# bzhangGo/zero

Measured on AMD Instinct MI355X. Metric: src+tgt tokens/sec training, Transformer-base d=512 L=6, higher is better.
Workload: dtype bf16; 1 GPU; Transformer-base (d=512, L=6+6, F=2048, h=8, V=32000) training step, B=64 x (src 64 + tgt 64) tokens per GPU, dropout 0.10, label_smooth 0.1, fwd+bwd+allreduce+Adam; model_name=transformer, parallelism=dp1, hip_graph=whole step

## Files before the change

### include/zero_hip.h

```cpp
#ifndef ZERO_HIP_H_
#define ZERO_HIP_H_

#include <stddef.h>
#include <stdint.h>

#ifdef __cplusplus
extern "C" {
#endif

typedef void* zk_stream_t;

int zk_version(void);
const char* zk_last_error_string(void);

size_t zk_gemm_workspace(int M, int N, int K);
size_t zk_gemm_workspace_split(int M, int N, int splits);
int zk_gemm_parts(const void* A, const void* B, float* parts, int M, int N, int K, int lda, int ldb, int ta, int tb,
                  int splits, int* nparts_out, zk_stream_t stream);
size_t zk_gemm_add_ln_workspace(int rows, int N);
int zk_ln_epoch_bump(uint32_t* epoch, zk_stream_t stream);
int zk_gemm_add_ln(const void* A, const void* B, int M, int N, int K, int lda, int ldb, const float* bias,
                   const void* residual, int ldr, float drop_p, const uint64_t* seed, uint32_t sid, const float* gamma,
                   const float* beta, float eps, void* s_out, void* y, float* mean, float* rstd, void* slots,
                   size_t slots_bytes, const uint32_t* epoch, uint32_t site, int* err, zk_stream_t stream);
// ... 97 lines not shown
int zk_ce_fused(const float* logits, const int* ids, const float* w, float* ce_out, void* dlogits, int rows,
                int V, int ld, float label_smooth, zk_stream_t stream);
int zk_target_stats(const int* ids, float* mask, float* w, int B, int L, float loss_scale, zk_stream_t stream);
int zk_loss_reduce(const float* ce, const int* ids, float* per_sample, float* loss, int B, int L,
                   zk_stream_t stream);
int zk_make_mask(const int* ids, float* mask, int n, zk_stream_t stream);
size_t zk_batch_prep_workspace(int rows);
int zk_batch_prep(const int* src_ids, const int* tgt_ids, int B, int Ls, int Lt, int* src_rows, int* src_seg,
                  int* src_uid, int* src_n, int* tgt_rows, int* tgt_seg, int* tgt_uid, int* tgt_n, float* smask,
                  float* tmask, float* tw, float loss_scale, int max_id, void* scratch, size_t scratch_bytes,
                  zk_stream_t stream);
int zk_copy_many(void* const* dsts, const void* const* srcs, const size_t* nbytes, int n, zk_stream_t stream);
int zk_all_equal(const int* ids, int n, int value, int* flag, zk_stream_t stream);

int zk_aan_fwd(const void* x, const float* mask, void* cat, int B, int L, int H, int use_mask,
               zk_stream_t stream);
int zk_add_bf16(void* out, int ldo, const void* a, int lda, const void* b, int ldb, int rows, int cols,
                zk_stream_t stream);
int zk_aan_bwd(const void* dcat, const void* dxg, const void* dyg, const void* ds, const float* mask, void* dx,
               int B, int L, int H, int use_mask, zk_stream_t stream);
int zk_aan_gate_fwd(const void* z, const void* cat, void* out, int rows, int H, zk_stream_t stream);
int zk_aan_gate_bwd(const void* dg, const void* z, const void* cat, void* dz, void* dxg, void* dyg, int rows,
                    int H, zk_stream_t stream);

size_t zk_norm_workspace(void);
int zk_l2norm(const float* x, size_t n, float scale, float* out, void* workspace, size_t ws_bytes,
              zk_stream_t stream);
int zk_adam(float* p, const float* g, float* m, float* v, void* shadow_bf16, size_t n, float* hyper,
            float* pnorm_out, void* workspace, size_t ws_bytes, zk_stream_t stream);
size_t zk_adam_step_workspace(void);
int zk_adam_step(float* p, const float* g, float* m, float* v, void* shadow_bf16, size_t n, float* hyper,
                 float* pnorm_out, uint64_t* seed, int norm_free, const int* skip_word, void* workspace, size_t ws_bytes,
                 zk_stream_t stream);
int zk_norm_flag(float* hyper, zk_stream_t stream);
int zk_cast_f32_bf16(const float* x, void* y, size_t n, zk_stream_t stream);
int zk_cast_bf16_f32(const void* x, float* y, size_t n, zk_stream_t stream);
int zk_zero(void* p, size_t bytes, zk_stream_t stream);
size_t zk_rows_payload_bytes(int R, int H, int bf16);
int zk_transpose_bf16(const void* src, int ld_src, void* dst, int ld_dst, int rows, int cols, zk_stream_t stream);
int zk_rows_pack(float* dtable, const int* uid, const int* n_uniq_dev, void* out, int R, int H, int out_bf16,
                 int clear_rows, zk_stream_t stream);
int zk_rows_scatter_add(float* dtable, const void* payload, int R, int H, int in_bf16, int vocab_rows,
                        zk_stream_t stream);
uint32_t zk_crc32c(const void* data, size_t n, uint32_t crc);
int zk_spin(uint32_t usec, zk_stream_t stream);
int zk_tune(int key, int value);
int zk_ema(float* ema, const float* p, const float* hyper, size_t n, zk_stream_t stream);
int zk_axpby_f32(float* y, const float* x, float a, float b, size_t n, zk_stream_t stream);

int zk_comm_available(void);
int zk_comm_unique_id(void* id128);
int zk_comm_init(const void* id128, int nranks, int rank, void** comm_out);
int zk_comm_destroy(void* comm);
int zk_comm_size(const void* comm);
int zk_comm_allreduce(void* comm, void* buf, size_t count, int dtype, zk_stream_t stream);
int zk_comm_allreduce_multi(void* comm, void* const* bufs, const size_t* counts, int n, int dtype,
                            zk_stream_t stream);
int zk_comm_allgather(void* comm, const void* send, void* recv, size_t count, int dtype, zk_stream_t stream);
int zk_flag_add(void* flag, zk_stream_t stream);
int zk_flag_wait(const void* flag, unsigned long long target, int* err, zk_stream_t stream);

int zk_dropout_mask(float* out, size_t n, float drop_p, const uint64_t* seed, uint32_t sid, zk_stream_t stream);
int zk_seed_advance(uint64_t* seed, uint64_t inc, zk_stream_t stream);

size_t zk_beam_topk_workspace(int B, int K, int k2);
int zk_beam_topk(const float* logits, const float* prev_log_probs, float* topk_scores, int* topk_index, int B,
// ... 152 lines not shown
```

### zero_amd/csrc/zk_elem.hip

```cpp
#include "zk_common.h"
#include "zk_ln_dev.h"
#ifdef ZK_STEP_STAMPS
__device__ unsigned long long zk_step_stamp_buf[2 * 4096];
__device__ unsigned int zk_step_stamp_n[2];
extern "C" int zk_step_stamps_read(unsigned long long* out, unsigned int* n2) {
  if (hipMemcpyFromSymbol(out, HIP_SYMBOL(zk_step_stamp_buf), sizeof(unsigned long long) * 2 * 4096) != hipSuccess) return 1;
  return (int)hipMemcpyFromSymbol(n2, HIP_SYMBOL(zk_step_stamp_n), sizeof(unsigned int) * 2);
}
extern "C" int zk_step_stamps_reset(void) {
  unsigned int z[2] = {0, 0};
  return (int)hipMemcpyToSymbol(HIP_SYMBOL(zk_step_stamp_n), z, sizeof(z));
}
#endif
#include <cstring>
#include <mutex>
#include <stdarg.h>
#include <stdio.h>
#include <unordered_map>

thread_local char zk_err_buf[512] = {0};
int zk_set_error(int code, const char* fmt, ...) {
  va_list ap;
  va_start(ap, fmt);
  vsnprintf(zk_err_buf, sizeof(zk_err_buf), fmt, ap);
// ... 1058 lines not shown
    dx[j] = g[j] * si;
    dy[j] = g[j] * sf;
  }
  *reinterpret_cast<uint4*>(dz + r * 2 * H + c) = pack8(dzi);
  *reinterpret_cast<uint4*>(dz + r * 2 * H + H + c) = pack8(dzf);
  *reinterpret_cast<uint4*>(dxg + r * H + c) = pack8(dx);
  *reinterpret_cast<uint4*>(dyg + r * H + c) = pack8(dy);
}

__global__ void __launch_bounds__(256) k_sumsq_partial(const float* __restrict__ x, size_t n,
                                                       float* __restrict__ partials) {
  __shared__ float sm[8];
  float acc = 0.f;
  const size_t n4 = n / 4;
  const float4* x4 = reinterpret_cast<const float4*>(x);
  for (size_t i = (size_t)blockIdx.x * 256 + threadIdx.x; i < n4; i += (size_t)gridDim.x * 256) {
    const float4 v = x4[i];
    acc += v.x * v.x + v.y * v.y + v.z * v.z + v.w * v.w;
  }
  for (size_t i = n4 * 4 + (size_t)blockIdx.x * 256 + threadIdx.x; i < n; i += (size_t)gridDim.x * 256)
    acc += x[i] * x[i];
  acc = block_sum<4>(acc, sm);
  if (threadIdx.x == 0) partials[blockIdx.x] = acc;
}
__global__ void __launch_bounds__(256) k_norm_final(const float* __restrict__ partials, int n, float scale,
                                                    float* __restrict__ out) {
  __shared__ float sm[8];
  float acc = 0.f;
  for (int i = threadIdx.x; i < n; i += 256) acc += partials[i];
  acc = block_sum<4>(acc, sm);
  if (threadIdx.x == 0) out[0] = scale * sqrtf(acc);
}

template <bool GSQ, int U = 1, bool CONTIG = false>
__global__ void __launch_bounds__(256) k_adam(float* __restrict__ p, const float* __restrict__ g,
                                              float* __restrict__ m, float* __restrict__ v,
                                              bf16_t* __restrict__ shadow, size_t n,
                                              float* __restrict__ hyper, float* __restrict__ psq,
                                              float* __restrict__ gsq, uint64_t* __restrict__ seed,
                                              const int* __restrict__ skip_word = nullptr, int nt = 0) {
  __shared__ float sm_[8];
  float pacc = 0.f;
  float gacc = 0.f;
  const float lr = hyper[0], b1 = hyper[1], b2 = hyper[2], eps = hyper[3];
  const float gs = hyper[4], clip = hyper[5], gnorm = hyper[6];
  if (seed != nullptr && blockIdx.x == 0 && threadIdx.x == 0) *seed += 1;
  if (skip_word != nullptr && *skip_word != 0) {
    if (threadIdx.x == 0) {
      if (psq != nullptr) psq[blockIdx.x] = 0.f;
      if (GSQ && gsq != nullptr) gsq[blockIdx.x] = __builtin_nanf("");
      if (!GSQ && blockIdx.x == 0) { hyper[7] = 1.f; hyper[10] += 1.f; }
    }
    return;
  }
  float f = gs;
  if (!GSQ) {
    if (!(gnorm == gnorm) || fabsf(gnorm) == INFINITY || (hyper[9] > 0.f && gnorm > hyper[9])) {
      if (blockIdx.x == 0 && threadIdx.x == 0) { hyper[7] = 1.f; hyper[10] += 1.f; }
      return;
    }
    if (blockIdx.x == 0 && threadIdx.x == 0) hyper[7] = 0.f;
    if (clip > 0.f) f *= clip / fmaxf(gnorm, clip);
  }
  const size_t n4 = n / 4;
  const bool contig = CONTIG;
  constexpr int UU = U;
// ... 45 lines not shown
          reinterpret_cast<float4*>(p)[i] = pp[u];
          reinterpret_cast<float4*>(m)[i] = mm[u];
          reinterpret_cast<float4*>(v)[i] = vv[u];
        }
        if (shadow != nullptr) {
          if (nt & 4) {
            zk_u32x2 sh2; sh2.x = pack2bf(P[0], P[1]); sh2.y = pack2bf(P[2], P[3]);
            __builtin_nontemporal_store(sh2, reinterpret_cast<zk_u32x2*>(shadow) + i);
          } else {
            reinterpret_cast<uint2*>(shadow)[i] = make_uint2(pack2bf(P[0], P[1]), pack2bf(P[2], P[3]));
          }
        }
      }
    }
  }
  for (size_t i = n4 * 4 + (size_t)blockIdx.x * 256 + threadIdx.x; i < n; i += (size_t)gridDim.x * 256) {
    const float gj = g[i] * f;
    if (GSQ) gacc += gj * gj;
    pacc += p[i] * p[i];
    m[i] = b1 * m[i] + (1.f - b1) * gj;
    v[i] = b2 * v[i] + (1.f - b2) * gj * gj;
    p[i] -= lr * m[i] / (sqrtf(v[i]) + eps);
    if (shadow != nullptr) shadow[i] = f2bf(p[i]);
  }
  if (psq != nullptr) {
    pacc = block_sum<4>(pacc, sm_);
    if (threadIdx.x == 0) psq[blockIdx.x] = pacc;
  }
  if (GSQ && gsq != nullptr) {
    gacc = block_sum<4>(gacc, sm_);
    if (threadIdx.x == 0) gsq[blockIdx.x] = gacc;
  }
}
__global__ void __launch_bounds__(256) k_norm_final2(const float* __restrict__ psq, const float* __restrict__ gsq,
                                                     int n, float* __restrict__ hyper, float* __restrict__ pnorm_out) {
  __shared__ float sm[8];
  float a = 0.f, b = 0.f;
  for (int i = threadIdx.x; i < n; i += 256) { a += gsq[i]; if (psq != nullptr) b += psq[i]; }
  a = block_sum<4>(a, sm);
  b = block_sum<4>(b, sm);
  if (threadIdx.x == 0) {
    const float gn = sqrtf(a);
    hyper[6] = gn;
    const bool bad = !(gn == gn) || fabsf(gn) == INFINITY;
    hyper[7] = bad ? 1.f : 0.f;
    if (bad) hyper[10] += 1.f;
    if (pnorm_out != nullptr) pnorm_out[0] = sqrtf(b);
#ifdef ZK_STEP_STAMPS
    {
      const unsigned int i_ = atomicAdd(&zk_step_stamp_n[1], 1u);
      if (i_ < 4096) zk_step_stamp_buf[4096 + i_] = __builtin_amdgcn_s_memrealtime();
    }
#endif
  }
}
__global__ void k_norm_flag(float* __restrict__ hyper) {
  const float gn = hyper[6];
  const bool bad = !(gn == gn) || fabsf(gn) == INFINITY;
  hyper[7] = bad ? 1.f : 0.f;
  if (bad) hyper[10] += 1.f;
}

__global__ void __launch_bounds__(256) k_cast_f32_bf16(const float* __restrict__ x, bf16_t* __restrict__ y, size_t n) {
  const size_t n4 = n / 4;
  for (size_t i = (size_t)blockIdx.x * 256 + threadIdx.x; i < n4; i += (size_t)gridDim.x * 256) {
    const float4 v = reinterpret_cast<const float4*>(x)[i];
    reinterpret_cast<uint2*>(y)[i] = make_uint2(pack2bf(v.x, v.y), pack2bf(v.z, v.w));
  }
  for (size_t i = n4 * 4 + (size_t)blockIdx.x * 256 + threadIdx.x; i < n; i += (size_t)gridDim.x * 256)
    y[i] = f2bf(x[i]);
}
__global__ void __launch_bounds__(256) k_cast_bf16_f32(const bf16_t* __restrict__ x, float* __restrict__ y, size_t n) {
  for (size_t i = (size_t)blockIdx.x * 256 + threadIdx.x; i < n; i += (size_t)gridDim.x * 256)
    y[i] = bf2f(x[i]);
}
__global__ void __launch_bounds__(256) k_axpy_f32(float* __restrict__ y, const float* __restrict__ x, float a,
                                                  float by, size_t n) {
  for (size_t i = (size_t)blockIdx.x * 256 + threadIdx.x; i < n; i += (size_t)gridDim.x * 256)
    y[i] = by * y[i] + a * x[i];
}
__global__ void __launch_bounds__(256) k_ema(float* __restrict__ ema, const float* __restrict__ p,
                                             const float* __restrict__ hyper, size_t n) {
  const float gnorm = hyper[6], d = hyper[8];
  if (!(gnorm == gnorm) || fabsf(gnorm) == INFINITY || (hyper[9] > 0.f && gnorm > hyper[9])) return;
  const size_t n4 = n / 4;
  for (size_t i = (size_t)blockIdx.x * 256 + threadIdx.x; i < n4; i += (size_t)gridDim.x * 256) {
// ... 465 lines not shown
}
size_t zk_adam_step_workspace(void) { return 2 * 2048 * sizeof(float); }
int zk_adam_step(float* p, const float* g, float* m, float* v, void* shadow, size_t n, float* hyper,
                 float* pnorm_out, uint64_t* seed, int norm_free, const int* skip_word, void* workspace, size_t ws_bytes,
                 hipStream_t stream) {
  ZK_CHECK_ARG((((uintptr_t)p | (uintptr_t)g | (uintptr_t)m | (uintptr_t)v) & 15) == 0,
               "zk_adam_step: buffers must be 16-byte aligned");
  ZK_CHECK_ARG(ws_bytes >= zk_adam_step_workspace(), "zk_adam_step: workspace too small");
  ZK_CHECK_ARG(hyper != nullptr, "zk_adam_step: hyper is required");
  if (n == 0) return 0;
  const int grid = flat_grid(n, 4);
  float* psq = (float*)workspace;
  float* gsq = psq + 2048;
  if (norm_free) {
    const int gb = g_tune[10] > 0 && g_tune[10] <= 2048 ? (grid < g_tune[10] ? grid : g_tune[10]) : grid;
#define ZK_ADAM_L(...) hipLaunchKernelGGL((k_adam<__VA_ARGS__>), dim3(gb), dim3(256), 0, stream, p, g, m, v, (bf16_t*)shadow, n, hyper, psq, gsq, seed, skip_word, g_tune[18])
    if (g_tune[9] == 1) ZK_ADAM_L(true, 1, true);
    else if (g_tune[9] == 2) ZK_ADAM_L(true, 2, true);
    else if (g_tune[9] == 4) ZK_ADAM_L(true, 4, true);
    else ZK_ADAM_L(true, 1, false);
#undef ZK_ADAM_L
    ZK_LAUNCH_CHECK();
    hipLaunchKernelGGL(k_norm_final2, dim3(1), dim3(256), 0, stream, (const float*)psq, (const float*)gsq, gb, hyper,
                       pnorm_out);
  } else {
    hipLaunchKernelGGL(k_adam<false>, dim3(grid), dim3(256), 0, stream, p, g, m, v, (bf16_t*)shadow, n, hyper, psq,
                       (float*)nullptr, seed, skip_word);
    ZK_LAUNCH_CHECK();
    if (pnorm_out) hipLaunchKernelGGL(k_norm_final, dim3(1), dim3(256), 0, stream, (const float*)psq, grid, 1.f, pnorm_out);
  }
  ZK_LAUNCH_CHECK();
  return 0;
}
int zk_norm_flag(float* hyper, hipStream_t stream) {
  ZK_CHECK_ARG(hyper != nullptr, "zk_norm_flag: hyper is required");
  hipLaunchKernelGGL(k_norm_flag, dim3(1), dim3(1), 0, stream, hyper);
  ZK_LAUNCH_CHECK();
  return 0;
}

int zk_cast_f32_bf16(const float* x, void* y, size_t n, hipStream_t stream) {
  if (n == 0) return 0;
  ZK_CHECK_ARG(((uintptr_t)x & 15) == 0 && ((uintptr_t)y & 7) == 0, "zk_cast_f32_bf16: misaligned");
  hipLaunchKernelGGL(k_cast_f32_bf16, dim3(flat_grid(n, 4)), dim3(256), 0, stream, x, (bf16_t*)y, n);
  ZK_LAUNCH_CHECK();
  return 0;
}
int zk_cast_bf16_f32(const void* x, float* y, size_t n, hipStream_t stream) {
  if (n == 0) return 0;
  hipLaunchKernelGGL(k_cast_bf16_f32, dim3(flat_grid(n, 1)), dim3(256), 0, stream, (const bf16_t*)x, y, n);
  ZK_LAUNCH_CHECK();
  return 0;
}
int zk_axpby_f32(float* y, const float* x, float a, float b, size_t n, hipStream_t stream) {
  if (n == 0) return 0;
  hipLaunchKernelGGL(k_axpy_f32, dim3(flat_grid(n, 1)), dim3(256), 0, stream, y, x, a, b, n);
  ZK_LAUNCH_CHECK();
  return 0;
}
int zk_ema(float* ema, const float* p, const float* hyper, size_t n, hipStream_t stream) {
  if (n == 0) return 0;
  if ((reinterpret_cast<uintptr_t>(ema) | reinterpret_cast<uintptr_t>(p)) & 15)
    return zk_set_error(-1, "zk_ema: buffers must be 16-byte aligned");
  hipLaunchKernelGGL(k_ema, dim3(flat_grid(n, 4)), dim3(256), 0, stream, ema, p, hyper, n);
  ZK_LAUNCH_CHECK();
  return 0;
// ... 136 lines not shown
```

### zero_amd/main.py

```python

import os
import time

import torch

from zero_amd import lrs
from zero_amd.models import model as model_registry
from zero_amd.models import load_all
from zero_amd.utils import parallel
from zero_amd.utils.cycle import TrainOp
from zero_amd.hip import ZeroHipError


def tower_train_graph(train_features, graph, params, reducer=None):
    out = graph.train_fn(train_features, params, on_ready=reducer.ready if reducer is not None else None)
    return out["loss"], out


def tower_score_graph(eval_features, graph, params):
    return graph.score_fn(eval_features, params)["score"]


def tower_infer_graph(eval_features, graph, params):
    from zero_amd.search import beam_search
# ... 158 lines not shown
                loss = self._step_static(True)
            cur.wait_stream(ws)
            return loss
        eng = self.core.eng
        cur = torch.cuda.current_stream(eng.device)
        ws = eng.work_stream
        ws.wait_stream(cur)
        with torch.cuda.stream(ws):
            loss = self._step_accumulate(features)
        cur.wait_stream(ws)
        return loss

    def _step_staged(self, staged, hstage, scale):
        eng = self.core.eng
        extra = self.train_op.hyper_pairs(hstage) + [(self._commit_reached.view(torch.float32), hstage[11:12])]
        fast = parallel.world_size() == 1 and not self.force_segmented and \
            os.environ.get("ZERO_HIP_COMMIT_IN_GRAPH", "1") != "0"
        key = ("stg", staged["B"], staged["Ls"], staged.get("Lt", 0))
        self._check_graph_cache()
        probe = None
        if fast:
            probe = self.core.commit(staged, extra=extra, launch=False)
            fast = eng.copy_many_fits(probe[1])
        g = self._graphs.pop(key, None) if fast else None
        if g is None:
            if fast:
                self._graphs[key] = "warm"
            self.batch = self.core.commit(staged, extra=extra)
            self._declare_sparse(self.batch)
            return self._step_static(not fast, scale=scale)
        if g == "warm":
            def body():
                self.batch = self.core.commit(staged, extra=extra)
                self._train_and_update(scale)
            g = eng.graph_capture(body)
        else:
            self.batch, pairs = probe
            if not eng.graph_set_copy_many(g, pairs):
                raise ZeroHipError("Trainer.step: the commit of a batch no longer fits one zk_copy_many launch")
        self._graphs[key] = g
        self._declare_sparse(self.batch)
        eng.graph_launch(g)
        self.store.step += 1
        self.global_step += 1
        return eng.buf("loss", (1,), torch.float32)

    def _graph_run(self, key, body):
        eng = self.core.eng
        g = self._graphs.pop(key, None)
        if g is None:
            self._graphs[key] = "warm"
            body()
            return
        if g == "warm":
            g = eng.graph_capture(body)
        self._graphs[key] = g
        eng.graph_launch(g)

    def _step_accumulate(self, features):
        hp, eng = self.params, self.core.eng
        world = parallel.world_size()
        self._check_graph_cache()
        if self.cycle_counter == 0:
            self.train_op.zero()
        last = (self.cycle_counter + 1) >= hp.update_cycle
        self.lr.step(self.global_step)
        batch = self.prepare_static(features)
# ... 87 lines not shown
        if True:
            stream = torch.cuda.current_stream(eng.device).cuda_stream
            plan, mark = [], [0]

            def begin():
                lib.call("zk_graph_begin", stream)
                mark[0] = lib.ncalls

            def cut():
                ex = ctypes.c_void_p()
                lib.call("zk_graph_end", stream, ctypes.byref(ex))
                return ex

            def on_ready(k):
                if lib.ncalls == mark[0] and plan and plan[-1][0] == "ready":
                    plan[-1][1].append(k)
                    return
                plan.append(("graph", cut()))
                plan.append(("ready", [k]))
                begin()

            begin()
            try:
                self.graph.train_fn(self.batch, hp, on_ready=on_ready)
            finally:
                plan.append(("graph", cut()))
            begin()
            try:
                self.train_op.launch_update(scale)
            finally:
                plan.append(("update", cut()))
            return plan

    def _train_and_update(self, scale):
        self.graph.train_fn(self.batch, self.params)
        self.train_op.launch_update(scale)

    def prepare_static(self, features):
        src, tgt = features["source"], features["target"]
        m = self.pad_len
        if m > 1:
            from zero_amd.models._core import trim_columns
            src, tgt = (trim_columns(np.asarray(t.cpu() if torch.is_tensor(t) else t)) for t in (src, tgt))
            src = np.pad(src, ((0, 0), (0, -src.shape[1] % m)))
            tgt = np.pad(tgt, ((0, 0), (0, -tgt.shape[1] % m)))
            self.batch = self.core.upload(src, tgt, trim=False)
            self._declare_sparse(self.batch)
            return self.batch
        self.batch = self.core.upload(src, tgt)
        self._declare_sparse(self.batch)
        return self.batch

    def step_static(self, use_graph=True):
        eng = self.core.eng
        cur = torch.cuda.current_stream(eng.device)
        ws = eng.work_stream
        if cur == ws:
            return self._step_static(use_graph)
        ws.wait_stream(cur)
        with torch.cuda.stream(ws):
            loss = self._step_static(use_graph)
        cur.wait_stream(ws)
        return loss

    MAX_GRAPHS = 96

    def _check_graph_cache(self):
        eng = self.core.eng
# ... 1 lines not shown
            for g in self._graphs.values():
                for h in (g if isinstance(g, list) else [("graph", g)]):
                    if h[0] in ("graph", "update") and not isinstance(h[1], str):
                        eng.lib.call("zk_graph_destroy", h[1])
            self._graphs = {}
            self._graph_gen = eng.realloc_gen
        while len(self._graphs) > self.MAX_GRAPHS:
            key = next(iter(self._graphs))
            g = self._graphs.pop(key)
            for h in (g if isinstance(g, list) else [("graph", g)]):
                if h[0] in ("graph", "update") and not isinstance(h[1], str):
                    eng.lib.call("zk_graph_destroy", h[1])

    def _step_static(self, use_graph, scale=None):
        hp = self.params
        assert hp.update_cycle == 1, "captured step supports update_cycle == 1"
        world = parallel.world_size()
        eng = self.core.eng
        self._check_graph_cache()
        if scale is None:
            self.lr.step(self.global_step)
            self.train_op.count = 0
            scale = self.train_op.set_hyper(self.lr.get_lr(), world)
        if world == 1 and use_graph and not self.force_segmented:
            key = (self.batch["B"], self.batch["Ls"], self.batch["Lt"])
            g = self._graphs.pop(key, None)
            if g is not None:
                self._graphs[key] = g
            if g is None:
                self._graphs[key] = "warm"
                return self._step_static(False, scale=scale)
            if g == "warm":
                def body():
                    self._train_and_update(scale)
                g = eng.graph_capture(body)
                self._graphs[key] = g
            eng.graph_launch(g)
        elif use_graph and (world > 1 or self.force_segmented):
            self._step_segmented(scale)
        elif world > 1:
            self.graph.train_fn(self.batch, hp, on_ready=self.reducer.ready)
            self._reduced_update(scale, None)
        else:
            self._train_and_update(scale)
        self.store.step += 1
        self.global_step += 1
        return eng.buf("loss", (1,), torch.float32)


import logging
import os
import time

import numpy as np

log = logging.getLogger("zero_amd")


def _restore(trainer, saver, path=None):
    from zero_amd.utils.saver import assign_tensors
    tensors = saver.restore(path)
    if tensors is None:
        return False
    got, missing, step = assign_tensors(trainer.store, trainer.params.scope_name or "model", tensors)
    for name in missing:
        log.warning("%s is missed", name)
    if step is not None:
# ... 240 lines not shown
```

### zero_amd/models/_core.py

```python

import os

import numpy as np
import torch

from zero_amd.func import Engine, Mat
from zero_amd.variables import get_store

BF16 = torch.bfloat16
F32 = torch.float32


def trim_columns(ids):
    ids = np.asarray(ids)
    keep = (ids != 0).any(axis=0)
    if keep.size:
        keep[0] = True
    return np.ascontiguousarray(ids[:, keep])


class TransformerCore(object):
    def __init__(self, params, model_name, store=None, device=None):
        self.hp = params
        self.model = model_name
# ... 16 lines not shown
            raise NotImplementedError("Not supported: {}".format(params.strategies))
        shared = params.shared_source_target_embedding
        self.src_emb = "embedding" if shared else "src_embedding"
        self.tgt_emb = "embedding" if shared else "tgt_embedding"
        if shared:
            self.soft_emb = "embedding"
        else:
            self.soft_emb = "tgt_embedding" if params.shared_target_softmax_embedding else "softmax_embedding"
        self.V = params.tgt_vocab.size()
        self.Vpad = self.store.pshape[self.soft_emb][0]
        self.group_wgrad = True
        import torch.distributed as _dist
        _multi = (_dist.is_available() and _dist.is_initialized() and _dist.get_world_size() > 1) or \
            os.environ.get("ZERO_HIP_FORCE_SEGMENTED", "0") != "0"
        self.group_layers = int(os.environ.get("ZERO_HIP_GROUP_LAYERS", "2" if _multi else "6"))
        self.group_all = not _multi
        self.wgrad_tile = (256, 256, 0) if self.group_all else (128, 256)
        self._pending_wgrads = []
        self._pending_colsums = []
        self._pending_lnred = []
        self._ln_bwd_done = {}
        self._ln_next = None
        self._pending_rpr = []
        self._pending_adds = []
        self._mem_segs = []
        self.kseg_mem = True
        self.logits_tile256 = True
        self.attn_oproj = os.environ.get("ZERO_HIP_ATTN_OPROJ", "auto").lower()
        self._red_id = 0
        self.sync_ln_mode = os.environ.get("ZERO_HIP_SYNC_LN", "1") != "0"
        self.merge_small = os.environ.get("ZERO_HIP_MERGE_SMALL", "1") != "0"
        if self.eng.device.type == "cuda":
            self.eng.lib.raw("zk_tune")(16, 0 if self.merge_small else 1)
        self.sync_ln_bwd = os.environ.get("ZERO_HIP_SYNC_LN", "1") != "fwd"
        self.sync_attn = os.environ.get("ZERO_HIP_SYNC_LN", "1") not in ("noattn", "fwd", "0")
        self.proj_attn = os.environ.get("ZERO_HIP_PROJ_ATTN", "1") != "0"
        self._sync_ln = False

    def _use_oproj(self, B):
        if self.attn_oproj in ("0", "1"):
            return self.attn_oproj == "1"
        return (not self.rpr) and self.H <= 512 and B * self.nh <= 512

    def _flush_wgrads(self):
        if self._pending_wgrads:
            probs = self._pending_wgrads
            self._pending_wgrads = []
            self.eng.gemm_grouped(probs, 1, 0, tile=self.wgrad_tile)
        if self._pending_colsums or self._pending_lnred or self._pending_rpr:
            cs, ln, rp = self._pending_colsums, self._pending_lnred, self._pending_rpr
            self._pending_colsums, self._pending_lnred, self._pending_rpr = [], [], []
            self.eng.reductions_grouped(cs, ln, rp)
        if self._pending_adds:
            adds = self._pending_adds
            self._pending_adds = []
            for dst, src in adds:
                self._accumulate(dst, src)

    def _defer_rpr(self):
        return self.rpr and self.group_wgrad and self.eng.gemm_impl == 0

    def _use_kseg(self):
        return self.kseg_mem and self.H % 64 == 0 and self.eng.gemm_impl == 0

    def _finish_mem_grad(self, d_mem):
        segs, self._mem_segs = self._mem_segs, []
# ... 521 lines not shown
                                      "backward are not built")
        ls = self.hp.label_smooth if label_smooth is None else label_smooth
        self._sync_ln = self.sync_ln_mode and self.eng.gemm_impl == 0 and self.H % 64 == 0 and \
            self.H <= 1024 and self.F % 64 == 0 and not self.fixup and self.eng.sync_ln_usable()
        pair_embeds = self.merge_small and "tgt" in batch
        if self._sync_ln and not pair_embeds:
            self.eng.ln_epoch_bump()
        self._embeds_done = False
        if pair_embeds:
            e_, H_ = self.eng, self.H
            e_.embed_fwd_pair(batch["src"], self.store.s(self.src_emb), e_.mat("enc.x0", batch["B"] * batch["Ls"], H_),
                              batch["Ls"], 9001, batch["tgt"], self.store.s(self.tgt_emb),
                              e_.mat("dec.x0", batch["B"] * batch["Lt"], H_), batch["Lt"], 9002, self.b("bias"), batch["B"], H_,
                              drop_p=self.hp.dropout if train else 0.0, bump_epoch=self._sync_ln)
            self._embeds_done = True
        try:
            enc, smask = self.encode(batch, train, save)
            feat, tmask, w = self.decode_train(batch, enc, smask, train, save)
        finally:
            self._embeds_done = False
        loss, per_sample, logits, dlogits = self.loss_head(batch, feat, w, ls, save)
        self._sync_ln = False
        self._ctx = (batch, enc, smask, feat, tmask, dlogits)
        return loss, per_sample, logits

    def backward(self, on_ready=None):
        e, hp, H = self.eng, self.hp, self.H
        if on_ready is None:
            on_ready = lambda key: None
        batch, enc, smask, feat, tmask, dlogits = self._ctx
        B, Ls, Lt = batch["B"], batch["Ls"], batch["Lt"]
        Ts, Tt = B * Ls, B * Lt
        st = self.store
        if self.src_emb != self.soft_emb:
            e.zero(st.g(self.src_emb))
        if self.tgt_emb != self.soft_emb and self.tgt_emb != self.src_emb:
            e.zero(st.g(self.tgt_emb))
        E = self.W(self.soft_emb)
        P = [e.mat("gd.p0", Tt, H), e.mat("gd.p1", Tt, H)]
        cur = 0
        e.gemm(dlogits, E, P[cur], Tt, H, self.Vpad, 0, 0)
        gE = self.gW(self.soft_emb)
        if self.group_wgrad and e.gemm_impl == 0:
            self._pending_wgrads.append((dlogits, feat, gE, self.Vpad, H, Tt, None, None, None))
        else:
            e.gemm(dlogits, feat, gE, self.Vpad, H, Tt, 1, 0)
        d_enc = e.mat("g.denc", Ts, H)
        if not self._use_kseg():
            e.zero(d_enc.t)
        NE = hp.num_encoder_layer

        def layer_input(side, l, kind):
            if side == "d":
                order = ([] if self.fuse else ["aa"] if self.aan else ["sa"]) + ["ca", "ff"]
            else:
                order = ["sa", "ff"]
            i = order.index(kind)
            if i > 0:
                return e.mat("%s%d.%s.o" % (side, l, order[i - 1]), Tt if side == "d" else Ts, H)
            if l > 0:
                return e.mat("%s%d.ff.o" % (side, l - 1), Tt if side == "d" else Ts, H)
            return e.mat("dec.x0" if side == "d" else "enc.x0", Tt if side == "d" else Ts, H)

        fuse_ln_bwd = self.sync_ln_mode and self.sync_ln_bwd and self.group_wgrad and e.gemm_impl == 0 and \
            H % 64 == 0 and H <= 1024 and not self.fuse and e.sync_ln_usable()

        def ln_below(side, l, kind):
            if not fuse_ln_bwd:
                return None
# ... 85 lines not shown
            self._self_attn_bwd(Q[cur], layer_input("e", l, "sa"), B, Ls, pre + "/self_attention", "e%d.sa" % l,
                                smask, False, 100 * l + 1, "e", other)
            Q[cur ^ 1] = other
            cur ^= 1
            self._ln_next = None
            ready_e.append(pre)
            if (not self.group_all and len(ready_e) >= self.group_layers) or l == 0:
                self._flush_wgrads()
                for key in ready_d + ready_e:
                    on_ready(key)
                ready_d, ready_e = [], []
        dxs = Q[cur]
        pair = self.group_all and self.merge_small and self.src_emb != self.tgt_emb
        if self.group_all:
            if ready_d:
                self._flush_wgrads()
                for key in ready_d:
                    on_ready(key)
            if not pair:
                tgt_embed_grads()
                tables_ready()

        def src_embed_grads():
            e.embed_bwd_sorted(batch["src_sort"], dxs, st.g(self.src_emb), H,
                               accumulate=(self.src_emb == self.tgt_emb), drop_p=hp.dropout, sid=9001)
            e.colsum(dxs, st.g("bias"), skip_L=0, accumulate=True, drop_p=hp.dropout, sid=9001)
            on_ready("bias")
            on_ready(self.src_emb)

        def both_embed_grads():
            e.embed_bwd_sorted_pair(batch["tgt_sort"], dxt, st.g(self.tgt_emb), self.tgt_emb == self.soft_emb, 9002,
                                    batch["src_sort"], dxs, st.g(self.src_emb), False, 9001, H, drop_p=hp.dropout)
            e.colsum_pair(dxt, Lt, 9002, dxs, 0, 9001, st.g("bias"), drop_p=hp.dropout)
        if pair:
            both_embed_grads()
            tables_ready()
            on_ready("bias")
            on_ready(self.src_emb)
        else:
            src_embed_grads()
```

### zero_amd/utils/cycle.py

```python

import math

import torch

from zero_amd import hip


class TrainOp(object):
    def __init__(self, store, params, engine):
        self.store, self.hp, self.eng = store, params, engine
        dev = store.device
        self.hyper = torch.zeros(12, dtype=torch.float32, device=dev)
        if getattr(params, "safe_nan", False) and getattr(params, "gnorm_upper_bound", 0.) > 0.:
            self.hyper[9] = float(params.gnorm_upper_bound)
        from zero_amd.utils.queuer import PinnedRing
        self._pins = PinnedRing(dev)
        self.ema = None
        self._backup = None
        if getattr(params, "ema_decay", -1.) > 0.:
            self.ema = store.master.clone()
        self.pnorm = torch.zeros(1, dtype=torch.float32, device=dev)
        self.count = 0
        _lib = hip.lib()
        self._ws = torch.empty(max(_lib.query("zk_norm_workspace") * 2, _lib.query("zk_adam_step_workspace")),
# ... 26 lines not shown
    def set_hyper(self, lr, world=1, dst=None, seq=None):
        hyper = self.hyper if dst is None else dst
        hp = self.hp
        t = self.store.step + 1
        lr_t = lr * math.sqrt(1.0 - hp.beta2 ** t) / (1.0 - hp.beta1 ** t)
        clip = hp.clip_grad_norm or None
        clip = float(clip) if isinstance(clip, float) else 0.0
        scale = 1.0 / (float(world) * float(hp.loss_scale) * float(self.count + 1))
        import numpy as _np
        if seq is not None:
            v = _np.zeros(12, dtype=_np.float32)
            v[:6] = [lr_t, hp.beta1, hp.beta2, hp.epsilon, scale, clip]
            if self.ema is not None:
                t_ = self.store.step + 1
                v[8] = min(float(hp.ema_decay), (1.0 + t_) / (10.0 + t_))
            v[11:12] = _np.array([seq], dtype=_np.int32).view(_np.float32)
            self._pins.put(hyper[:12], v)
            return scale
        self._pins.put(hyper[:6], _np.array([lr_t, hp.beta1, hp.beta2, hp.epsilon, scale, clip], dtype=_np.float32))
        if self.ema is not None:
            self._pins.put(hyper[8:9], _np.array([min(float(hp.ema_decay), (1.0 + t) / (10.0 + t))],
                                                      dtype=_np.float32))
        return scale

    def hyper_pairs(self, staged):
        pairs = [(self.hyper[:6], staged[:6])]
        if self.ema is not None:
            pairs.append((self.hyper[8:9], staged[8:9]))
        return pairs

    def launch_update(self, scale, advance_seed=True):
        st, lib, s = self.store, self.eng.lib, self.eng.stream
        norm_free = self.can_update_by_range()
        if not norm_free:
            lib.call("zk_l2norm", st.grad.data_ptr(), st.numel, scale, self.hyper.data_ptr() + 6 * 4,
                     self._ws.data_ptr(), self._ws.numel(), s)
        lib.call("zk_adam_step", st.master.data_ptr(), st.grad.data_ptr(), st.m.data_ptr(), st.v.data_ptr(),
                 st.shadow.data_ptr(), st.numel, self.hyper.data_ptr(), self.pnorm.data_ptr(),
                 self.eng.seed.data_ptr() if advance_seed else None, 1 if norm_free else 0,
                 self.eng.sync_ln_err_ptr(),
                 self._ws.data_ptr(), self._ws.numel(), s)
        if self.ema is not None:
            lib.call("zk_ema", self.ema.data_ptr(), st.master.data_ptr(), self.hyper.data_ptr(), st.numel, s)

    def can_update_by_range(self):
        hp = self.hp
        clip = hp.clip_grad_norm or None
        return not isinstance(clip, float) and not getattr(hp, "safe_nan", False)

    def begin_update_by_range(self):
        self.hyper[6:7].fill_(1.0)

    def launch_update_range(self, lo, hi):
        st, lib, s = self.store, self.eng.lib, self.eng.stream
        n = hi - lo
        lib.call("zk_adam", st.master.data_ptr() + lo * 4, st.grad.data_ptr() + lo * 4, st.m.data_ptr() + lo * 4,
                 st.v.data_ptr() + lo * 4, st.shadow.data_ptr() + lo * 2, n, self.hyper.data_ptr(), None, None, 0, s)

    def finish_update_by_range(self, scale):
        st, lib, s = self.store, self.eng.lib, self.eng.stream
        nb = self._ws.numel() // 2
        lib.call("zk_l2norm", st.grad.data_ptr(), st.numel, scale, self.hyper.data_ptr() + 6 * 4,
                 self._ws.data_ptr(), nb, s)
        lib.call("zk_norm_flag", self.hyper.data_ptr(), s)
        lib.call("zk_l2norm", st.master.data_ptr(), st.numel, 1.0, self.pnorm.data_ptr(), self._ws.data_ptr() + nb, nb, s)
        if self.ema is not None:
# ... 37 lines not shown
```

Before: 2.123 million src+tgt tokens/s.

## Fuse sparse embedding gradient gather into the Adam step kernel

Instead of zeroing the full source/target embedding gradient tables and scatter-adding token gradients into them, the Adam kernel now gathers each embedding row's gradient directly from the sorted token output gradients, reapplying dropout and embedding scale, via a precomputed row map. This removes the zero-fill and the scatter pass over the large vocab tables within the captured whole-step graph. The norm reduction is folded into a last-block finalisation inside the same kernel. It adds per-element branching and gather reads in the optimizer, and only works on the norm-free path.

```diff
diff --git a/include/zero_hip.h b/include/zero_hip.h
--- a/include/zero_hip.h
+++ b/include/zero_hip.h
@@ -153,6 +153,13 @@
 int zk_adam_step(float* p, const float* g, float* m, float* v, void* shadow_bf16, size_t n, float* hyper,
                  float* pnorm_out, uint64_t* seed, int norm_free, const int* skip_word, void* workspace, size_t ws_bytes,
                  zk_stream_t stream);
+int zk_adam_step_rows(float* p, const float* g, float* m, float* v, void* shadow_bf16, size_t n, float* hyper,
+                      float* pnorm_out, uint64_t* seed, const int* skip_word, void* workspace, size_t ws_bytes,
+                      size_t lo_a, size_t hi_a, int H_a, int stride_a, int dense_a, const int* rows_a, const int* seg_a,
+                      const int* uid_a, const int* n_a, int max_a, const void* dout_a, int ld_a, uint32_t sid_a,
+                      int* rowmap_a, size_t lo_b, size_t hi_b, int H_b, int stride_b, int dense_b, const int* rows_b,
+                      const int* seg_b, const int* uid_b, const int* n_b, int max_b, const void* dout_b, int ld_b,
+                      uint32_t sid_b, int* rowmap_b, float emb_scale, float drop_p, zk_stream_t stream);
 int zk_norm_flag(float* hyper, zk_stream_t stream);
 int zk_cast_f32_bf16(const float* x, void* y, size_t n, zk_stream_t stream);
 int zk_cast_bf16_f32(const void* x, float* y, size_t n, zk_stream_t stream);
diff --git a/zero_amd/csrc/zk_elem.hip b/zero_amd/csrc/zk_elem.hip
--- a/zero_amd/csrc/zk_elem.hip
+++ b/zero_amd/csrc/zk_elem.hip
@@ -1114,6 +1114,167 @@
   if (threadIdx.x == 0) out[0] = scale * sqrtf(acc);
 }
 
+struct AdamRowsTable {
+  size_t lo, hi;
+  const int* rows_sorted; const int* seg; const int* uid; const int* n_uniq_dev;
+  const bf16_t* dout;
+  int* rowmap;
+  int H, stride, ld, nrows, max_uniq, dense;
+  uint32_t sid;
+};
+struct AdamRowsArgs { AdamRowsTable t[2]; float scale; uint32_t thr; float inv_keep; };
+
+__device__ __forceinline__ void zk_drop_scale4(uint64_t seed, uint32_t sid, uint64_t base, uint32_t thr, float inv_keep,
+                                               float (&m)[4]) {
+  const uint32_t t16 = thr >> 16;
+#pragma unroll
+  for (int k = 0; k < 2; ++k) {
+    const uint32_t r = zk_drop_bits(seed, sid, (base >> 1) + k);
+    m[2 * k] = (r & 0xffffu) >= t16 ? inv_keep : 0.f;
+    m[2 * k + 1] = (r >> 16) >= t16 ? inv_keep : 0.f;
+  }
+}
+__device__ __forceinline__ float4 adam_rows_sum4(const AdamRowsTable& T, int u, int c, float scale, uint32_t thr,
+                                                 float inv_keep, uint64_t seed) {
+#pragma clang fp contract(off)
+  const int s0 = T.seg[u], s1 = T.seg[u + 1];
+  float acc[4] = {0.f, 0.f, 0.f, 0.f};
+  int rr[16];
+#pragma unroll
+  for (int j = 0; j < 16; ++j) rr[j] = s0 + j < s1 ? T.rows_sorted[s0 + j] : 0;
+  for (int k0 = s0; k0 < s1; k0 += 16) {
+    const int nb = min(16, s1 - k0);
+    uint2 raw[16];
+    int nx[16];
+#pragma unroll
+    for (int j = 0; j < 16; ++j)
+      if (j < nb) raw[j] = *reinterpret_cast<const uint2*>(T.dout + (size_t)rr[j] * T.ld + c);
+#pragma unroll
+    for (int j = 0; j < 16; ++j) nx[j] = k0 + 16 + j < s1 ? T.rows_sorted[k0 + 16 + j] : 0;
+#pragma unroll
+    for (int j = 0; j < 16; ++j) {
+      if (j < nb) {
+        float x[4] = {bf2f((bf16_t)(raw[j].x & 0xffffu)), bf2f((bf16_t)(raw[j].x >> 16)),
+                      bf2f((bf16_t)(raw[j].y & 0xffffu)), bf2f((bf16_t)(raw[j].y >> 16))};
+        if (thr) {
+          float dm[4];
+          zk_drop_scale4(seed, T.sid, (uint64_t)rr[j] * T.H + c, thr, inv_keep, dm);
+#pragma unroll
+          for (int q = 0; q < 4; ++q) x[q] *= dm[q];
+        }
+#pragma unroll
+        for (int q = 0; q < 4; ++q) acc[q] += x[q];
+      }
+    }
+#pragma unroll
+    for (int j = 0; j < 16; ++j) rr[j] = nx[j];
+  }
+  return make_float4(acc[0] * scale, acc[1] * scale, acc[2] * scale, acc[3] * scale);
+}
+__device__ __forceinline__ float4 adam_rows_grad4(const AdamRowsArgs& R, size_t i, const float* __restrict__ g,
+                                                  uint64_t seed) {
+#pragma clang fp contract(off)
+  const size_t e = 4 * i;
+  int u = -2, dense = 0;
+  float4 s = make_float4(0.f, 0.f, 0.f, 0.f);
+#pragma unroll
+  for (int t = 0; t < 2; ++t) {
+    const AdamRowsTable& T = R.t[t];
+    if (e >= T.lo && e < T.hi) {
+      const uint32_t rel = (uint32_t)(e - T.lo);
+      const uint32_t row = rel / (uint32_t)T.stride;
+      const int c = (int)(rel - row * (uint32_t)T.stride);
+      if (c < T.H) {
+        u = T.rowmap[row];
+        dense = T.dense;
+        if (u >= 0) s = adam_rows_sum4(T, u, c, R.scale, R.thr, R.inv_keep, seed);
+      }
+    }
+  }
+  if (u != -2 && !dense) return s;
+  const zk_f32x4 t4 = __builtin_nontemporal_load(reinterpret_cast<const zk_f32x4*>(g) + i);
+  if (u < 0) return make_float4(t4.x, t4.y, t4.z, t4.w);
+  s.x += t4.x; s.y += t4.y; s.z += t4.z; s.w += t4.w;
+  return s;
+}
+
+template <int U, bool CONTIG>
+__device__ __forceinline__ void adam_rows_pass(float* __restrict__ p, const float* __restrict__ g, float* __restrict__ m,
+                                          float* __restrict__ v, bf16_t* __restrict__ shadow, size_t n, float lr, float b1,
+                                          float b2, float eps, float f, int nt, const AdamRowsArgs& R, uint64_t seed,
+                                          float& pacc, float& gacc) {
+  const size_t n4 = n / 4;
+  const bool contig = CONTIG;
+  constexpr int UU = U;
+  const size_t per_block = ((n4 + gridDim.x - 1) / gridDim.x + 255) / 256 * 256;
+  const size_t stride = contig ? 256 : (size_t)gridDim.x * 256;
+  const size_t ibeg = contig ? (size_t)blockIdx.x * per_block + threadIdx.x : (size_t)blockIdx.x * 256 + threadIdx.x;
+  const size_t iend = contig ? min(n4, (size_t)(blockIdx.x + 1) * per_block) : n4;
+  for (size_t i0 = ibeg; i0 < iend; i0 += UU * stride) {
+    float4 pp[UU], gg[UU], mm[UU], vv[UU];
+#pragma unroll
+    for (int u = 0; u < UU; ++u) {
+      const size_t i = i0 + u * stride;
+      if (i < iend) {
+        if (nt & 2) {
+          const zk_f32x4 a4 = __builtin_nontemporal_load(reinterpret_cast<const zk_f32x4*>(p) + i);
+          const zk_f32x4 b4 = __builtin_nontemporal_load(reinterpret_cast<const zk_f32x4*>(m) + i);
+          const zk_f32x4 c4 = __builtin_nontemporal_load(reinterpret_cast<const zk_f32x4*>(v) + i);
+          pp[u] = make_float4(a4.x, a4.y, a4.z, a4.w);
+          mm[u] = make_float4(b4.x, b4.y, b4.z, b4.w);
+          vv[u] = make_float4(c4.x, c4.y, c4.z, c4.w);
+        } else {
+          pp[u] = reinterpret_cast<float4*>(p)[i];
+          mm[u] = reinterpret_cast<float4*>(m)[i];
+          vv[u] = reinterpret_cast<float4*>(v)[i];
+        }
+        gg[u] = adam_rows_grad4(R, i, g, seed);
+      }
+    }
+#pragma unroll
+    for (int u = 0; u < UU; ++u) {
+      const size_t i = i0 + u * stride;
+      if (i < iend) {
+        pacc += pp[u].x * pp[u].x + pp[u].y * pp[u].y + pp[u].z * pp[u].z + pp[u].w * pp[u].w;
+        float* P = &pp[u].x; const float* G = &gg[u].x; float* M = &mm[u].x; float* Vv = &vv[u].x;
+#pragma unroll
+        for (int j = 0; j < 4; ++j) {
+          const float gj = G[j] * f;
+          gacc += gj * gj;
+          M[j] = __builtin_fmaf(b1, M[j], (1.f - b1) * gj);
+          Vv[j] = __builtin_fmaf(gj, (1.f - b2) * gj, b2 * Vv[j]);
+          P[j] -= lr * M[j] / (sqrtf(Vv[j]) + eps);
+        }
+        if (nt & 1) {
+          __builtin_nontemporal_store((zk_f32x4){pp[u].x, pp[u].y, pp[u].z, pp[u].w}, reinterpret_cast<zk_f32x4*>(p) + i);
+          __builtin_nontemporal_store((zk_f32x4){mm[u].x, mm[u].y, mm[u].z, mm[u].w}, reinterpret_cast<zk_f32x4*>(m) + i);
+          __builtin_nontemporal_store((zk_f32x4){vv[u].x, vv[u].y, vv[u].z, vv[u].w}, reinterpret_cast<zk_f32x4*>(v) + i);
+        } else {
+          reinterpret_cast<float4*>(p)[i] = pp[u];
+          reinterpret_cast<float4*>(m)[i] = mm[u];
+          reinterpret_cast<float4*>(v)[i] = vv[u];
+        }
+        if (shadow != nullptr) {
+          if (nt & 4) {
+            zk_u32x2 sh2; sh2.x = pack2bf(P[0], P[1]); sh2.y = pack2bf(P[2], P[3]);
+            __builtin_nontemporal_store(sh2, reinterpret_cast<zk_u32x2*>(shadow) + i);
+          } else {
+            reinterpret_cast<uint2*>(shadow)[i] = make_uint2(pack2bf(P[0], P[1]), pack2bf(P[2], P[3]));
+          }
+        }
+      }
+    }
+  }
+  for (size_t i = n4 * 4 + (size_t)blockIdx.x * 256 + threadIdx.x; i < n; i += (size_t)gridDim.x * 256) {
+    const float gj = g[i] * f;
+    gacc += gj * gj;
+    pacc += p[i] * p[i];
+    m[i] = __builtin_fmaf(1.f - b1, gj, b1 * m[i]);
+    v[i] = __builtin_fmaf(gj, (1.f - b2) * gj, b2 * v[i]);
+    p[i] -= lr * m[i] / (sqrtf(v[i]) + eps);
+    if (shadow != nullptr) shadow[i] = f2bf(p[i]);
+  }
+}
 template <bool GSQ, int U = 1, bool CONTIG = false>
 __global__ void __launch_bounds__(256) k_adam(float* __restrict__ p, const float* __restrict__ g,
                                               float* __restrict__ m, float* __restrict__ v,
@@ -1225,6 +1386,20 @@
     if (threadIdx.x == 0) gsq[blockIdx.x] = gacc;
   }
 }
+__device__ __forceinline__ void norm_final2_book(float a, float b, float* __restrict__ hyper, float* __restrict__ pnorm_out) {
+  const float gn = sqrtf(a);
+  hyper[6] = gn;
+  const bool bad = !(gn == gn) || fabsf(gn) == INFINITY;
+  hyper[7] = bad ? 1.f : 0.f;
+  if (bad) hyper[10] += 1.f;
+  if (pnorm_out != nullptr) pnorm_out[0] = sqrtf(b);
+#ifdef ZK_STEP_STAMPS
+  {
+    const unsigned int i_ = atomicAdd(&zk_step_stamp_n[1], 1u);
+    if (i_ < 4096) zk_step_stamp_buf[4096 + i_] = __builtin_amdgcn_s_memrealtime();
+  }
+#endif
+}
 __global__ void __launch_bounds__(256) k_norm_final2(const float* __restrict__ psq, const float* __restrict__ gsq,
                                                      int n, float* __restrict__ hyper, float* __restrict__ pnorm_out) {
   __shared__ float sm[8];
@@ -1245,6 +1420,59 @@
       if (i_ < 4096) zk_step_stamp_buf[4096 + i_] = __builtin_amdgcn_s_memrealtime();
     }
 #endif
+  }
+}
+
+__global__ void __launch_bounds__(256) k_adam_rows_map(AdamRowsArgs R) {
+  const AdamRowsTable& T = R.t[blockIdx.y];
+  if (T.nrows <= 0) return;
+  const int nu = max(0, min(*T.n_uniq_dev, T.max_uniq));
+  for (int r = blockIdx.x * 256 + threadIdx.x; r < T.nrows; r += gridDim.x * 256) {
+    int lo = 0, hi = nu;
+    while (lo < hi) {
+      const int mid = (lo + hi) >> 1;
+      if (T.uid[mid] < r) lo = mid + 1; else hi = mid;
+    }
+    T.rowmap[r] = (lo < nu && T.uid[lo] == r) ? lo : -1;
+  }
+}
+__device__ unsigned int zk_adam_rows_done = 0;
+template <int U, bool CONTIG>
+__global__ void __launch_bounds__(256) k_adam_rows(float* __restrict__ p, const float* __restrict__ g, float* __restrict__ m,
+                                                   float* __restrict__ v, bf16_t* __restrict__ shadow, size_t n,
+                                                   float* __restrict__ hyper, float* psq, float* gsq, float* __restrict__ pnorm_out,
+                                                   uint64_t* seed, const int* __restrict__ skip_word, int nt, AdamRowsArgs R) {
+  __shared__ float sm_[8];
+  __shared__ int last_;
+  float pacc = 0.f, gacc = 0.f;
+  const float lr = hyper[0], b1 = hyper[1], b2 = hyper[2], eps = hyper[3], gs = hyper[4];
+  if (skip_word != nullptr && *skip_word != 0) {
+    gacc = __builtin_nanf("");
+  } else {
+    adam_rows_pass<U, CONTIG>(p, g, m, v, shadow, n, lr, b1, b2, eps, gs, nt, R, R.thr ? *seed : 0, pacc, gacc);
+    pacc = block_sum<4>(pacc, sm_);
+    gacc = block_sum<4>(gacc, sm_);
+  }
+  if (threadIdx.x == 0) {
+    __hip_atomic_store(psq + blockIdx.x, pacc, __ATOMIC_RELAXED, __HIP_MEMORY_SCOPE_AGENT);
+    __hip_atomic_store(gsq + blockIdx.x, gacc, __ATOMIC_RELAXED, __HIP_MEMORY_SCOPE_AGENT);
+    __threadfence();
+    last_ = atomicAdd(&zk_adam_rows_done, 1u) == gridDim.x - 1;
+  }
+  __syncthreads();
+  if (!last_) return;
+  __threadfence();
+  float a = 0.f, b = 0.f;
+  for (int i = threadIdx.x; i < (int)gridDim.x; i += 256) {
+    a += __hip_atomic_load(gsq + i, __ATOMIC_RELAXED, __HIP_MEMORY_SCOPE_AGENT);
+    b += __hip_atomic_load(psq + i, __ATOMIC_RELAXED, __HIP_MEMORY_SCOPE_AGENT);
+  }
+  a = block_sum<4>(a, sm_);
+  b = block_sum<4>(b, sm_);
+  if (threadIdx.x == 0) {
+    norm_final2_book(a, b, hyper, pnorm_out);
+    if (seed != nullptr) *seed += 1;
+    zk_adam_rows_done = 0;
   }
 }
 __global__ void k_norm_flag(float* __restrict__ hyper) {
@@ -1776,6 +2004,63 @@
   ZK_LAUNCH_CHECK();
   return 0;
 }
+static int adam_rows_table(AdamRowsTable& T, const char* which, size_t n, size_t lo, size_t hi, int H, int stride, int dense,
+                           const int* rows, const int* seg, const int* uid, const int* n_uniq, int max_uniq, const void* dout,
+                           int ld, uint32_t sid, int* rowmap) {
+  T = AdamRowsTable{};
+  if (hi <= lo) return 0;
+  ZK_CHECK_ARG(hi <= n && lo % 4 == 0 && hi % 4 == 0 && hi - lo < ((size_t)1 << 31),
+               "zk_adam_step_rows: table %s: bad range [%zu, %zu) of %zu", which, lo, hi, n);
+  ZK_CHECK_ARG(H > 0 && H % 4 == 0 && stride >= H && stride % 4 == 0 && ld >= H && ld % 4 == 0,
+               "zk_adam_step_rows: table %s: H=%d stride=%d ld=%d must be multiples of 4, H <= stride, H <= ld", which, H, stride, ld);
+  ZK_CHECK_ARG(rows && seg && uid && n_uniq && dout && rowmap && max_uniq >= 0, "zk_adam_step_rows: table %s: missing argument", which);
+  ZK_CHECK_ARG(((uintptr_t)dout & 7) == 0, "zk_adam_step_rows: table %s: dout must be 8-byte aligned", which);
+  T.lo = lo; T.hi = hi; T.rows_sorted = rows; T.seg = seg; T.uid = uid; T.n_uniq_dev = n_uniq;
+  T.dout = (const bf16_t*)dout; T.rowmap = rowmap; T.H = H; T.stride = stride; T.ld = ld;
+  T.nrows = (int)((hi - lo + stride - 1) / stride); T.max_uniq = max_uniq; T.dense = dense ? 1 : 0; T.sid = sid;
+  return 0;
+}
+int zk_adam_step_rows(float* p, const float* g, float* m, float* v, void* shadow, size_t n, float* hyper,
+                      float* pnorm_out, uint64_t* seed, const int* skip_word, void* workspace, size_t ws_bytes,
+                      size_t lo_a, size_t hi_a, int H_a, int stride_a, int dense_a, const int* rows_a, const int* seg_a,
+                      const int* uid_a, const int* n_a, int max_a, const void* dout_a, int ld_a, uint32_t sid_a,
+                      int* rowmap_a, size_t lo_b, size_t hi_b, int H_b, int stride_b, int dense_b, const int* rows_b,
+                      const int* seg_b, const int* uid_b, const int* n_b, int max_b, const void* dout_b, int ld_b,
+                      uint32_t sid_b, int* rowmap_b, float emb_scale, float drop_p, hipStream_t stream) {
+  ZK_CHECK_ARG((((uintptr_t)p | (uintptr_t)g | (uintptr_t)m | (uintptr_t)v) & 15) == 0,
+               "zk_adam_step_rows: buffers must be 16-byte aligned");
+  ZK_CHECK_ARG(ws_bytes >= zk_adam_step_workspace(), "zk_adam_step_rows: workspace too small");
+  ZK_CHECK_ARG(hyper != nullptr, "zk_adam_step_rows: hyper is required");
+  ZK_CHECK_ARG(drop_p == 0.f || seed != nullptr, "zk_adam_step_rows: dropout needs a seed pointer");
+  AdamRowsArgs R;
+  if (adam_rows_table(R.t[0], "a", n, lo_a, hi_a, H_a, stride_a, dense_a, rows_a, seg_a, uid_a, n_a, max_a, dout_a, ld_a,
+                      sid_a, rowmap_a)) return -1;
+  if (adam_rows_table(R.t[1], "b", n, lo_b, hi_b, H_b, stride_b, dense_b, rows_b, seg_b, uid_b, n_b, max_b, dout_b, ld_b,
+                      sid_b, rowmap_b)) return -1;
+  ZK_CHECK_ARG(R.t[0].hi <= R.t[0].lo || R.t[1].hi <= R.t[1].lo || R.t[0].hi <= R.t[1].lo || R.t[1].hi <= R.t[0].lo,
+               "zk_adam_step_rows: the two table ranges overlap");
+  R.scale = emb_scale;
+  R.thr = drop_p > 0.f ? zk_drop_threshold(drop_p) : 0;
+  R.inv_keep = drop_p > 0.f ? 1.f / (1.f - drop_p) : 1.f;
+  if (n == 0) return 0;
+  const int mr = R.t[0].nrows > R.t[1].nrows ? R.t[0].nrows : R.t[1].nrows;
+  if (mr > 0) {
+    hipLaunchKernelGGL(k_adam_rows_map, dim3((mr + 255) / 256, 2), dim3(256), 0, stream, R);
+    ZK_LAUNCH_CHECK();
+  }
+  const int grid = flat_grid(n, 4);
+  float* psq = (float*)workspace;
+  float* gsq = psq + 2048;
+  const int gb = g_tune[10] > 0 && g_tune[10] <= 2048 ? (grid < g_tune[10] ? grid : g_tune[10]) : grid;
+#define ZK_ADAM_R(...) hipLaunchKernelGGL((k_adam_rows<__VA_ARGS__>), dim3(gb), dim3(256), 0, stream, p, g, m, v, (bf16_t*)shadow, n, hyper, psq, gsq, pnorm_out, seed, skip_word, g_tune[18], R)
+  if (g_tune[9] == 1) ZK_ADAM_R(1, true);
+  else if (g_tune[9] == 2) ZK_ADAM_R(2, true);
+  else if (g_tune[9] == 4) ZK_ADAM_R(4, true);
+  else ZK_ADAM_R(1, false);
+#undef ZK_ADAM_R
+  ZK_LAUNCH_CHECK();
+  return 0;
+}
 int zk_norm_flag(float* hyper, hipStream_t stream) {
   ZK_CHECK_ARG(hyper != nullptr, "zk_norm_flag: hyper is required");
   hipLaunchKernelGGL(k_norm_flag, dim3(1), dim3(1), 0, stream, hyper);
diff --git a/zero_amd/main.py b/zero_amd/main.py
--- a/zero_amd/main.py
+++ b/zero_amd/main.py
@@ -214,7 +214,7 @@
         if g == "warm":
             def body():
                 self.batch = self.core.commit(staged, extra=extra)
-                self._train_and_update(scale)
+                self._train_and_update(scale, captured=True)
             g = eng.graph_capture(body)
         else:
             self.batch, pairs = probe
@@ -368,8 +368,12 @@
                 plan.append(("update", cut()))
             return plan
 
-    def _train_and_update(self, scale):
-        self.graph.train_fn(self.batch, self.params)
+    def _train_and_update(self, scale, captured=False):
+        self.core.sparse_emb_step = captured and self.train_op.can_update_by_range()
+        try:
+            self.graph.train_fn(self.batch, self.params)
+        finally:
+            self.core.sparse_emb_step = False
         self.train_op.launch_update(scale)
 
     def prepare_static(self, features):
@@ -437,7 +441,7 @@
                 return self._step_static(False, scale=scale)
             if g == "warm":
                 def body():
-                    self._train_and_update(scale)
+                    self._train_and_update(scale, captured=True)
                 g = eng.graph_capture(body)
                 self._graphs[key] = g
             eng.graph_launch(g)
diff --git a/zero_amd/models/_core.py b/zero_amd/models/_core.py
--- a/zero_amd/models/_core.py
+++ b/zero_amd/models/_core.py
@@ -72,6 +72,8 @@
         self.merge_small = os.environ.get("ZERO_HIP_MERGE_SMALL", "1") != "0"
         if self.eng.device.type == "cuda":
             self.eng.lib.raw("zk_tune")(16, 0 if self.merge_small else 1)
+        self.sparse_emb = os.environ.get("ZERO_HIP_SPARSE_EMB", "1") != "0"
+        self.sparse_emb_step = False
         self.sync_ln_bwd = os.environ.get("ZERO_HIP_SYNC_LN", "1") != "fwd"
         self.sync_attn = os.environ.get("ZERO_HIP_SYNC_LN", "1") not in ("noattn", "fwd", "0")
         self.proj_attn = os.environ.get("ZERO_HIP_PROJ_ATTN", "1") != "0"
@@ -659,9 +661,14 @@
         B, Ls, Lt = batch["B"], batch["Ls"], batch["Lt"]
         Ts, Tt = B * Ls, B * Lt
         st = self.store
-        if self.src_emb != self.soft_emb:
+        sparse = self.sparse_emb and self.group_all and self.merge_small and self.src_emb != self.tgt_emb
+        if sparse:
+            rowmaps = [e.buf("adam.rowmap." + k, (st.pshape[k][0],), torch.int32) for k in (self.tgt_emb, self.src_emb)]
+        sparse = sparse and self.sparse_emb_step
+        e.sparse_emb_tables = None
+        if self.src_emb != self.soft_emb and not sparse:
             e.zero(st.g(self.src_emb))
-        if self.tgt_emb != self.soft_emb and self.tgt_emb != self.src_emb:
+        if self.tgt_emb != self.soft_emb and self.tgt_emb != self.src_emb and not sparse:
             e.zero(st.g(self.tgt_emb))
         E = self.W(self.soft_emb)
         P = [e.mat("gd.p0", Tt, H), e.mat("gd.p1", Tt, H)]
@@ -813,7 +820,15 @@
             e.embed_bwd_sorted_pair(batch["tgt_sort"], dxt, st.g(self.tgt_emb), self.tgt_emb == self.soft_emb, 9002,
                                     batch["src_sort"], dxs, st.g(self.src_emb), False, 9001, H, drop_p=hp.dropout)
             e.colsum_pair(dxt, Lt, 9002, dxs, 0, 9001, st.g("bias"), drop_p=hp.dropout)
-        if pair:
+        if pair and sparse:
+            e.sparse_emb_tables = ([(self.tgt_emb, self.tgt_emb == self.soft_emb, batch["tgt_sort"], dxt, 9002, rowmaps[0]),
+                                    (self.src_emb, self.src_emb == self.soft_emb, batch["src_sort"], dxs, 9001, rowmaps[1])],
+                                   float(H) ** 0.5, hp.dropout)
+            e.colsum_pair(dxt, Lt, 9002, dxs, 0, 9001, st.g("bias"), drop_p=hp.dropout)
+            tables_ready()
+            on_ready("bias")
+            on_ready(self.src_emb)
+        elif pair:
             both_embed_grads()
             tables_ready()
             on_ready("bias")
diff --git a/zero_amd/utils/cycle.py b/zero_amd/utils/cycle.py
--- a/zero_amd/utils/cycle.py
+++ b/zero_amd/utils/cycle.py
@@ -82,6 +82,26 @@
     def launch_update(self, scale, advance_seed=True):
         st, lib, s = self.store, self.eng.lib, self.eng.stream
         norm_free = self.can_update_by_range()
+        tabs = getattr(self.eng, "sparse_emb_tables", None)
+        self.eng.sparse_emb_tables = None
+        if tabs is not None:
+            if not (norm_free and advance_seed):
+                raise hip.ZeroHipError("launch_update: unscattered embedding gradients need the norm-free whole-step update")
+            (ta, tb), emb_scale, drop_p = tabs
+            args = []
+            for name, dense, sort, dout, sid, rowmap in (ta, tb):
+                rows, H = st.pshape[name]
+                lo = st.offsets[name]
+                args += [lo, lo + rows * H, H, H, 1 if dense else 0, sort["rows"].data_ptr(), sort["seg"].data_ptr(),
+                         sort["uid"].data_ptr(), sort["n"].data_ptr(), sort["max_uniq"], dout.ptr, dout.ld, sid,
+                         rowmap.data_ptr()]
+            lib.call("zk_adam_step_rows", st.master.data_ptr(), st.grad.data_ptr(), st.m.data_ptr(), st.v.data_ptr(),
+                     st.shadow.data_ptr(), st.numel, self.hyper.data_ptr(), self.pnorm.data_ptr(),
+                     self.eng.seed.data_ptr(), self.eng.sync_ln_err_ptr(), self._ws.data_ptr(), self._ws.numel(),
+                     *(args + [float(emb_scale), float(drop_p), s]))
+            if self.ema is not None:
+                lib.call("zk_ema", self.ema.data_ptr(), st.master.data_ptr(), self.hyper.data_ptr(), st.numel, s)
+            return
         if not norm_free:
             lib.call("zk_l2norm", st.grad.data_ptr(), st.numel, scale, self.hyper.data_ptr() + 6 * 4,
                      self._ws.data_ptr(), self._ws.numel(), s)
```

Measured after the change: 2.084 million src+tgt tokens/s. 0.982x the previous value.
